# poriya219/modulations

Hardware: NVIDIA B200
Metric: turbo_info_throughput_N212_R1/3_8it (higher is better)
Workload: dtype f32/f64

## Files before the change

### modulations_b200/csrc/decode_tpf.cu

```cuda
#include "common.cuh"
#include "tpf_core.cuh"
#include "tpf_dev.cuh"

namespace b200dvb {

namespace {

using namespace tpf;

constexpr int kW = kTpfWin;

__device__ unsigned long long g_tpf_cycles[8];

struct TpfArgs {
    TpfGeom g;
    int B, iterations, n_tiles, n_llr, vec4;
    double sf_inner, sf_last;
    const int16_t *tab;
    const void *llr;
    long long llr_stride;
    int32_t *bits;
    uint32_t *packed;
    const uint8_t *ref_bits;
    unsigned long long *counters;
    unsigned char *ws;
    float llr_scale;
};

struct Ctx {
    int N, M, T;
    int f, isb, lane;
    unsigned tq;
    unsigned ycol;
    float4 *srec;
    unsigned char *stage;
    const int16_t *perm, *inv;
    float4 *L1A, *L2A;
    double2 *Le, *LeF, *Yb;
    float4 *CK;
    unsigned long long pol;
    unsigned one;
    __device__ __forceinline__ float4 *wstore() const { return reinterpret_cast<float4 *>(stage); }
    __device__ __forceinline__ float4 *slotZ() const { return reinterpret_cast<float4 *>(stage + 8192); }
    __device__ __forceinline__ float4 *slotX() const { return reinterpret_cast<float4 *>(stage + 10240); }
};

__device__ __forceinline__ void smem_get(const Ctx &c, int k, float (&g)[8])
{
    const float4 lo = c.srec[((k - c.T) * 2) * 16 + c.f], hi = c.srec[((k - c.T) * 2 + 1) * 16 + c.f];
    g[0] = lo.x; g[1] = lo.y; g[2] = lo.z; g[3] = lo.w; g[4] = hi.x; g[5] = hi.y; g[6] = hi.z; g[7] = hi.w;
}
__device__ __forceinline__ void smem_put(const Ctx &c, int k, const float (&g)[8])
{
    c.srec[((k - c.T) * 2) * 16 + c.f] = make_float4(g[0], g[1], g[2], g[3]);
    c.srec[((k - c.T) * 2 + 1) * 16 + c.f] = make_float4(g[4], g[5], g[6], g[7]);
}

struct Buf { float a[8], b[8]; };
template <int KIND> __device__ __forceinline__ void pf_issue(const Ctx &c, int j, Buf &B)
{
    if (KIND == 0) tm_ld8(c.tq + 8u * j, B.a);
    if (KIND == 1) smem_get(c, c.isb ? c.N - 1 - j : j, B.a);
    if (KIND == 2) {
        const unsigned col = 8u * (c.N - 1 - j);
        tm_ld8_half(c.tq + col, B.b);
        tm_ld8_half(c.tq + (16u << 16) + col, B.a);
    }
}
template <int KIND> __device__ __forceinline__ void pf_complete(const Ctx &c, Buf &B, float (&g)[8])
{
    if (KIND == 0) tm_wait_ld(B.a);
    if (KIND == 2) { tm_wait_ld(B.a); tm_wait_ld(B.b); }
#pragma unroll
    for (int i = 0; i < 8; ++i) g[i] = (KIND == 2 && c.isb) ? B.b[i] : B.a[i];
}

__device__ __forceinline__ constexpr int apos(int p) { return (p >> 1) | ((p & 1) << 3); }
__device__ __forceinline__ void pass_out(const Ctx &c, const float (&v)[16], float (&n)[16])
{
#pragma unroll
    for (int p = 0; p < 16; ++p) n[p] = c.isb ? v[rho4(p)] : v[apos(p)];
}
__device__ __forceinline__ void ck_store(const Ctx &c, int slot, const float (&v)[16])
{
    float n[16];
    pass_out(c, v, n);
#pragma unroll
    for (int q = 0; q < 4; ++q)
        st_ws(c.CK + (slot * 4 + q) * 32 + c.lane, make_float4(n[4 * q], n[4 * q + 1], n[4 * q + 2], n[4 * q + 3]));
}

template <int KIND, bool CK>
__device__ __forceinline__ void pass_two(const Ctx &c, int j, int j1, Buf &B0, Buf &B1, float (&g)[8], float (&v)[16])
{
    pf_issue<KIND>(c, j + 1, B1);
    if (CK) ck_store(c, (c.M - j) / kW - 1, v);
    pass_step(v, g, c.isb);
    pf_complete<KIND>(c, B1, g);
    pf_issue<KIND>(c, min(j + 2, j1 - 1), B0);
    pass_step(v, g, c.isb);
    pf_complete<KIND>(c, B0, g);
}
template <int KIND, bool CKA, bool CKB>
__device__ __forceinline__ void pass_loop(const Ctx &c, int j0, int j1, Buf &B0, Buf &B1, float (&g)[8], float (&v)[16])
{
    int j = j0;
    for (; j + 4 <= j1; j += 4) {
        pass_two<KIND, CKA>(c, j, j1, B0, B1, g, v);
        pass_two<KIND, CKB>(c, j + 2, j1, B0, B1, g, v);
    }
    if (j < j1) pass_two<KIND, CKA>(c, j, j1, B0, B1, g, v);
}
template <int KIND, bool CKPT>
__device__ __forceinline__ void run_pass(const Ctx &c, int j0, int j1, float (&v)[16])
{
    static_assert(kW == 4, "checkpoints alternate between the step pairs of a four-step body");
    if (j0 >= j1) return;
    Buf B0, B1;
    float g[8];
    pf_issue<KIND>(c, j0, B0);
    pf_complete<KIND>(c, B0, g);
    if (!CKPT) { pass_loop<KIND, false, false>(c, j0, j1, B0, B1, g, v); return; }
    if (j0 == 0 && (c.M % kW) != 0) ck_store(c, c.M / kW, v);
    if (((c.M - j0) % kW) == 0) pass_loop<KIND, CKPT, false>(c, j0, j1, B0, B1, g, v);
    else                        pass_loop<KIND, false, CKPT>(c, j0, j1, B0, B1, g, v);
}

__device__ __forceinline__ void issue_ckpt(const Ctx &c, int slot)
{
    float4 *dst = (c.isb ? c.slotZ() : c.slotX()) + c.lane;
#pragma unroll
    for (int q = 0; q < 4; ++q) cpa16(dst + q * 32, c.CK + (slot * 4 + q) * 32 + c.lane, c.one);
}
template <bool ALPHA = false>
__device__ __forceinline__ void slot_get(const float4 *slot, int lane, float (&v)[16])
{
    constexpr int P[4] = {ALPHA ? apos(0) : 0, ALPHA ? apos(1) : 1, ALPHA ? apos(2) : 2, ALPHA ? apos(3) : 3};
#pragma unroll
    for (int q = 0; q < 4; ++q) {
        const float4 t = slot[q * 32 + lane];
        const int b = ALPHA ? 2 * q : 4 * q;
        v[b + P[0]] = t.x; v[b + P[1]] = t.y; v[b + P[2]] = t.z; v[b + P[3]] = t.w;
    }
}
template <bool ALPHA = false>
__device__ __forceinline__ void slot_put(float4 *slot, int lane, const float (&v)[16])
{
    constexpr int P[4] = {ALPHA ? apos(0) : 0, ALPHA ? apos(1) : 1, ALPHA ? apos(2) : 2, ALPHA ? apos(3) : 3};
#pragma unroll
    for (int q = 0; q < 4; ++q) {
        const int b = ALPHA ? 2 * q : 4 * q;
        slot[q * 32 + lane] = make_float4(v[b + P[0]], v[b + P[1]], v[b + P[2]], v[b + P[3]]);
    }
}

__device__ __forceinline__ void st256_f64(void *p, double a, double b, double c, double d)
{
    asm volatile("st.global.cg.v4.f64 [%0], {%1,%2,%3,%4};" :: "l"(p), "d"(a), "d"(b), "d"(c), "d"(d) : "memory");
}
__device__ __forceinline__ void ld256_f64(const void *p, double2 &lo, double2 &hi)
{
    asm volatile("ld.global.cg.v4.f64 {%0,%1,%2,%3}, [%4];" : "=d"(lo.x), "=d"(lo.y), "=d"(hi.x), "=d"(hi.y) : "l"(p) : "memory");
}
__device__ __forceinline__ unsigned char *y_entry(const Ctx &c, int k_even)
{
    return reinterpret_cast<unsigned char *>(c.Yb) + ((size_t)(k_even >> 1) * 16 + c.f) * 32;
}
struct YQ { double2 y[kW]; };
__device__ __forceinline__ void yq_load(const Ctx &c, int w0, int len, YQ &q)
{
    static_assert(kW == 4, "two 32-byte entries per window");
    ld256_f64(y_entry(c, w0), q.y[0], q.y[1]);
    ld256_f64(y_entry(c, len > 2 ? w0 + 2 : w0), q.y[2], q.y[3]);
}
__device__ __forceinline__ void yq_park(const Ctx &c, const YQ &q, int w0, int len, int ck_slot)
{

#pragma unroll
    for (int u = 0; u < kW; ++u)
        asm volatile("tcgen05.st.sync.aligned.32x32b.x4.b32 [%0], {%1,%2,%3,%4};"
                     :: "r"(c.tq + c.ycol + 4u * u), "r"(__double2loint(q.y[u].x)), "r"(__double2hiint(q.y[u].x)),
                        "r"(__double2loint(q.y[u].y)), "r"(__double2hiint(q.y[u].y)) : "memory");
    tm_wait_st();
    const int dir = (c.lane >> 3) & 1, pr = (c.lane >> 2) & 1, l16 = c.lane & 15;
    const int w0d = __shfl_sync(0xffffffffu, w0, dir << 4);
    const void *line = c.lane < 16
        ? static_cast<const void *>(reinterpret_cast<const unsigned char *>(c.Yb) + ((size_t)((w0d >> 1) + pr) * 16) * 32 + (c.lane & 3) * 128)
        : static_cast<const void *>(c.CK + (ck_slot * 4 + (l16 >> 2)) * 32 + (l16 & 3) * 8);
    if (c.lane < 16 ? 2 * pr < len : ck_slot >= 0) l2_discard(line);
}

struct Pend { float uv[4], y[4]; int idx; };
__device__ __forceinline__ void pend_flush(const Ctx &c, Pend &p, double sf, double2 *LeOut)
{
    double ea, eb;
    make_extrinsic(p.uv, __hiloint2double(__float_as_int(p.y[1]), __float_as_int(p.y[0])),
                   __hiloint2double(__float_as_int(p.y[3]), __float_as_int(p.y[2])), sf, ea, eb);
    if (p.idx >= 0) st_ws(LeOut + p.idx * 16 + c.f, make_double2(ea, eb));
    p.idx = -1;
}
template <bool TM>
__device__ __forceinline__ void window(const Ctx &c, int wa, int w0, int len, double sf,
                                       double2 *LeOut, int nslot, int nw0, int nlen, Pend &pend)
{
    Buf B;
    auto issue = [&](int u) {
        if (TM) { tm_ld8(c.tq + 8u * (wa + u), B.a); tm_ld8(c.tq + 8u * (wa + len - 1 - u), B.b); }
        else    smem_get(c, w0 + u, B.a);
    };
    auto complete = [&](float (&g)[8]) {
        if (TM) { tm_wait_ld(B.a); tm_wait_ld(B.b); }
#pragma unroll
        for (int i = 0; i < 8; ++i) g[i] = (TM && c.isb) ? B.b[i] : B.a[i];
    };
    YQ nq;
    if (nlen) yq_load(c, nw0, nlen, nq);
    float g[8];
    float4 *ws = c.wstore() + c.lane;
    {
        float Z[16];
        issue(len - 1);
        slot_get(c.slotZ(), c.lane, Z);
        complete(g);
        slot_put(ws + (len - 1) * 128, 0, Z);
        issue(len - 2);
        pend_flush(c, pend, sf, LeOut);
        bwd_step(Z, g);
        complete(g);
        for (int u = len - 2; u >= 0; --u) {
            slot_put(ws + u * 128, 0, Z);
            issue(u > 0 ? u - 1 : 0);
            bwd_step(Z, g);
            complete(g);
        }
        if (!c.isb) slot_put(c.slotZ(), c.lane, Z);
    }
    float X[16];
    slot_get<true>(c.slotX(), c.lane, X);
    if (nslot >= 0) issue_ckpt(c, nslot);
    cpa_commit();
    float yr[4], yn[4], uvp[4], zs[16];
    tm_ld4(c.tq + c.ycol, yr);
    issue(len > 1 ? 1 : 0);
    slot_get(ws, 0, zs);
    ext_step(X, zs, g, uvp);
    tm_wait_ld4(yr);
    complete(g);
    for (int u = 1; u < len; ++u) {
        tm_ld4(c.tq + c.ycol + 4u * u, yn);
        issue(u + 1 < len ? u + 1 : u);
        slot_get(ws + u * 128, 0, zs);
        float uv[4];
        ext_step(X, zs, g, uv);
        double ea, eb;
        make_extrinsic(uvp, __hiloint2double(__float_as_int(yr[1]), __float_as_int(yr[0])),
                       __hiloint2double(__float_as_int(yr[3]), __float_as_int(yr[2])), sf, ea, eb);
        st_ws(LeOut + (w0 + u - 1) * 16 + c.f, make_double2(ea, eb));
        tm_wait_ld4(yn);
        complete(g);
#pragma unroll
        for (int i = 0; i < 4; ++i) { uvp[i] = uv[i]; yr[i] = yn[i]; }
    }
#pragma unroll
    for (int i = 0; i < 4; ++i) { pend.uv[i] = uvp[i]; pend.y[i] = yr[i]; }
    pend.idx = w0 + len - 1;
    if (c.isb) slot_put<true>(c.slotX(), c.lane, X);
    if (nlen) yq_park(c, nq, nw0, nlen, nslot - 1);
}


__device__ __forceinline__ int lpos(const Ctx &c, int k, int fr) { return k < c.M ? k * 32 + fr : (c.N - 1 - k) * 32 + 16 + fr; }

struct Idx { int a, b; };
__device__ __forceinline__ void idx_get(const Ctx &c, int jn, const int16_t *tbl, Idx &x)
{
    jn = min(jn, c.M - 2);
    const int k0 = c.isb ? c.N - 1 - jn : jn, k1 = c.isb ? k0 - 1 : k0 + 1;
    x.a = tbl[k0]; x.b = tbl[k1];
}
__device__ __forceinline__ void prep_load_pair(const Ctx &c, unsigned char *slot, int jn, const float4 *Lsrc,
                                               const Idx &x, bool first)
{
    jn = min(jn, c.M - 2);
    const unsigned d = s_addr(slot) * c.one;
    const float4 *src = Lsrc + jn * 32 + c.lane;
    cpa16_stream_off<0, 0>(d, src, c.pol);
    cpa16_stream_off<1024, 512>(d, src, c.pol);
    if (!first) {
        cpa16_off<512, 0>(d, c.Le + x.a * 16 + c.f);
        cpa16_off<1536, 0>(d, c.Le + x.b * 16 + c.f);
    }
}
struct Raw { float4 xA, xB; double2 laA, laB; };
template <bool FIRST>
__device__ __forceinline__ void raw_get(const unsigned char *slot, Raw &r)
{
    r.xA = *reinterpret_cast<const float4 *>(slot);
    r.xB = *reinterpret_cast<const float4 *>(slot + 1024);
    r.laA = r.laB = make_double2(0.0, 0.0);
    if (!FIRST) {
        r.laA = *reinterpret_cast<const double2 *>(slot + 512);
        r.laB = *reinterpret_cast<const double2 *>(slot + 1536);
    }
}
struct PrepRec { float gA[8], gB[8]; };
__device__ __forceinline__ void prep_pair(const Ctx &c, const Raw &r, int jn, PrepRec &out)
{
    jn = min(jn, c.M - 2);
    const double2 YA = make_double2(d_add((double)r.xA.x, r.laA.x), d_add((double)r.xA.y, r.laA.y));
    const double2 YB = make_double2(d_add((double)r.xB.x, r.laB.x), d_add((double)r.xB.y, r.laB.y));
    make_record(YA.x, YA.y, r.xA.z, r.xA.w, out.gA);
    make_record(YB.x, YB.y, r.xB.z, r.xB.w, out.gB);
#ifndef TPF_ABL_NOY
    const int ke = c.isb ? c.N - 2 - jn : jn;
    st256_f64(y_entry(c, ke), c.isb ? YB.x : YA.x, c.isb ? YB.y : YA.y, c.isb ? YA.x : YB.x, c.isb ? YA.y : YB.y);
#endif
}
struct PrepState { PrepRec r; Raw raw; Idx ix; int ps; };
template <bool FIRST, bool TMST>
__device__ __forceinline__ void pass1a_pair(const Ctx &c, int jj, const float4 *Lsrc, const int16_t *tbl,
                                            int &ps, const PrepRec &in, PrepRec &out, const Raw &rin, Raw &rout,
                                            const Idx &xin, Idx &xout, float (&v)[16])
{
    const int N = c.N;
    unsigned char *slot = c.stage + c.lane * 16 + ps * 2048;
    cpa_wait<kRingPairs - 1>();
#ifndef TPF_ABL_NORAW
    raw_get<FIRST>(slot, rout);
#else
    rout = rin;
#endif
#ifndef TPF_ABL_NOCPA
    prep_load_pair(c, slot, jj + 4 + 2 * kRingPairs, Lsrc, xin, FIRST);
    cpa_commit();
    if (!FIRST) idx_get(c, jj + 6 + 2 * kRingPairs, tbl, xout);
#endif
    ps = ps == kRingPairs - 1 ? 0 : ps + 1;
#ifndef TPF_ABL_NOFP64
    prep_pair(c, rin, jj + 2, out);
#else
    out = in;
#endif
    const int k0 = c.isb ? N - 1 - jj : jj, k1 = c.isb ? N - 2 - jj : jj + 1;
#ifndef TPF_ABL_NOREC
    if (TMST) tm_st8(c.tq + 8u * jj, in.gA);
    else      smem_put(c, k0, in.gA);
#endif
    pass_step(v, in.gA, c.isb);
#ifndef TPF_ABL_NOREC
    if (TMST) tm_st8(c.tq + 8u * (jj + 1), in.gB);
    else      smem_put(c, k1, in.gB);
#endif
    pass_step(v, in.gB, c.isb);
}
template <bool FIRST, bool TMST>
__device__ __forceinline__ void pass1a_range(const Ctx &c, int j0, int j1, const float4 *Lsrc,
                                             const int16_t *tbl, PrepState &P, float (&v)[16])
{
    PrepRec Q;
    Raw RQ;
    Idx XQ = P.ix;
    int jj = j0;
    for (; jj + 4 <= j1; jj += 4) {
        pass1a_pair<FIRST, TMST>(c, jj, Lsrc, tbl, P.ps, P.r, Q, P.raw, RQ, P.ix, XQ, v);
        pass1a_pair<FIRST, TMST>(c, jj + 2, Lsrc, tbl, P.ps, Q, P.r, RQ, P.raw, XQ, P.ix, v);
    }
    if (jj < j1) {
        pass1a_pair<FIRST, TMST>(c, jj, Lsrc, tbl, P.ps, P.r, Q, P.raw, RQ, P.ix, XQ, v);
        P.r = Q;
        P.raw = RQ;
        P.ix = XQ;
    }
}

template <bool FIRST>
__device__ __forceinline__ void pass1a(const Ctx &c, bool second, float (&v)[16])
{
    const float4 *Lsrc = second ? c.L2A : c.L1A;
    const int16_t *tbl = second ? c.perm : c.inv;
    unsigned char *ring = c.stage + c.lane * 16;
    PrepState P;
    P.ix.a = P.ix.b = 0;
#pragma unroll 1
    for (int p = 0; p < kRingPairs; ++p) {
        if (!FIRST) idx_get(c, 2 * p, tbl, P.ix);
        prep_load_pair(c, ring + p * 2048, 2 * p, Lsrc, P.ix, FIRST);
        cpa_commit();
    }
    if (!FIRST) idx_get(c, 2 * kRingPairs, tbl, P.ix);
    cpa_wait<kRingPairs - 1>();
    raw_get<FIRST>(ring, P.raw);
    prep_pair(c, P.raw, 0, P.r);
    prep_load_pair(c, ring, 2 * kRingPairs, Lsrc, P.ix, FIRST);
    cpa_commit();
    if (!FIRST) idx_get(c, 2 * kRingPairs + 2, tbl, P.ix);
    cpa_wait<kRingPairs - 1>();
    raw_get<FIRST>(ring + 2048, P.raw);
    prep_load_pair(c, ring + 2048, 2 * kRingPairs + 2, Lsrc, P.ix, FIRST);
    cpa_commit();
    if (!FIRST) idx_get(c, 2 * kRingPairs + 4, tbl, P.ix);
    P.ps = 2 % kRingPairs;
    pass1a_range<FIRST, true>(c, 0, c.T, Lsrc, tbl, P, v);
    pass1a_range<FIRST, false>(c, c.T, c.M, Lsrc, tbl, P, v);
    cpa_wait<0>();
}

template <bool TIMED>
__device__ __forceinline__ void siso(const Ctx &c, bool second, bool first, bool last, double sf, long long (&ph)[8])
{
    long long tA = TIMED ? clock64() : 0;
    const int N = c.N, M = c.M, T = c.T, lane = c.lane;
    double2 *LeOut = last ? c.LeF : c.Le;
    float v[16];
#pragma unroll
    for (int s = 0; s < 16; ++s) v[s] = 0.f;
    if (first) pass1a<true>(c, second, v);
    else       pass1a<false>(c, second, v);
    tm_wait_st();
    __syncwarp();
    if (!first && !last)
        for (int i = lane; i < N * 2; i += 32) l2_discard(c.Le + i * 8);
    if (TIMED) { const long long t = clock64(); ph[1] += t - tA; tA = t; }
    run_pass<1, false>(c, M, N - T, v);
    run_pass<2, false>(c, N - T, N, v);
    if (TIMED) { const long long t = clock64(); ph[2] += t - tA; tA = t; }
    const int nfull = M / kW, rag = M % kW, nwin = nfull + (rag ? 1 : 0);
    auto win_w0 = [&](int i) { return i < nfull ? (c.isb ? M + i * kW : M - (i + 1) * kW) : (c.isb ? N - rag : 0); };
    auto win_len = [&](int i) { return i < nfull ? kW : rag; };
    {
        YQ q0;
        yq_load(c, win_w0(0), win_len(0), q0);
        run_pass<0, true>(c, 0, T, v);
        run_pass<1, true>(c, T, M, v);
        yq_park(c, q0, win_w0(0), win_len(0), -1);
    }
    if (TIMED) { const long long t = clock64(); ph[3] += t - tA; tA = t; }
    {
        float n[16];
        pass_out(c, v, n);
        slot_put(c.isb ? c.slotZ() : c.slotX(), lane ^ 16, n);
    }
    const int n_inner = (M - T) / kW;
    issue_ckpt(c, 0);
    cpa_commit();
    Pend pend;
#pragma unroll
    for (int i = 0; i < 4; ++i) pend.uv[i] = pend.y[i] = 0.f;
    pend.idx = -1;
    for (int i = 0; i < nwin; ++i) {
        cpa_wait<0>();
        __syncwarp();
        const int wa = i < nfull ? M - (i + 1) * kW : 0;
        const int nlen = i + 1 < nwin ? win_len(i + 1) : 0;
        const int nw0 = i + 1 < nwin ? win_w0(i + 1) : 0;
        if (i < n_inner) window<false>(c, wa, win_w0(i), win_len(i), sf, LeOut, nlen ? i + 1 : -1, nw0, nlen, pend);
        else             window<true>(c, wa, win_w0(i), win_len(i), sf, LeOut, nlen ? i + 1 : -1, nw0, nlen, pend);
        if (TIMED && i == n_inner - 1) { const long long t = clock64(); ph[4] += t - tA; tA = t; }
    }
    pend_flush(c, pend, sf, LeOut);
    cpa_wait<0>();
    __syncwarp();
    if (TIMED) { const long long t = clock64(); ph[5] += t - tA; tA = t; }
}

template <bool TIMED, class LlrT>
__global__ void __launch_bounds__(kTpfWarps * 32, 1)
tpf_kernel(const TpfArgs A)
{
    extern __shared__ __align__(16) unsigned char smem_raw[];
    const TpfGeom g = A.g;
    const int N = g.N;
    const int tid = threadIdx.x, lane = tid & 31, warp = tid >> 5;
    int16_t *tab = reinterpret_cast<int16_t *>(smem_raw);
    const int tab_bytes = ((2 * N * 2 + 15) / 16) * 16;
    unsigned *tmem_slot = reinterpret_cast<unsigned *>(smem_raw + tab_bytes);
    float4 *srec_all = reinterpret_cast<float4 *>(smem_raw + tab_bytes + 64);
    unsigned char *stage_all = reinterpret_cast<unsigned char *>(srec_all + (size_t)kTpfWarps * g.mid * 2 * 16);
    if (warp == 0) {
        asm volatile("tcgen05.alloc.cta_group::1.sync.aligned.shared::cta.b32 [%0], %1;"
                     ::"r"((unsigned)__cvta_generic_to_shared(tmem_slot)), "r"(g.tmem_cols) : "memory");
        asm volatile("tcgen05.relinquish_alloc_permit.cta_group::1.sync.aligned;" ::: "memory");
    }
    for (int i = tid; i < 2 * N; i += blockDim.x) tab[i] = A.tab[i];
    const unsigned mbar = (unsigned)__cvta_generic_to_shared(smem_raw + tab_bytes + 32 + 8 * warp);
    unsigned mphase = 0;
    if (lane == 0) { mbar_init(mbar, 1); mbar_fence_init(); }
    asm volatile("tcgen05.fence::before_thread_sync;" ::: "memory");
    __syncthreads();
    asm volatile("tcgen05.fence::after_thread_sync;" ::: "memory");
    const unsigned tmem_base = *tmem_slot;

    Ctx c;
    c.N = N; c.M = g.M; c.T = g.T;
    c.f = lane & 15; c.isb = lane >> 4; c.lane = lane;
    c.tq = tmem_base + (((unsigned)warp * 32u) << 16);
    c.ycol = 8u * g.T;
    c.srec = srec_all + (size_t)warp * g.mid * 2 * 16;
    {
        volatile unsigned *slots = reinterpret_cast<volatile unsigned *>(smem_raw + tab_bytes);
        if (lane == 0) { slots[4 + warp] = (unsigned)warp * kStageBytes; slots[1] = 1u; }
        __syncwarp();
        c.stage = stage_all + slots[4 + warp];
        c.one = slots[1];
        __syncwarp();
    }
    c.perm = tab; c.inv = tab + N;
    const int wg = blockIdx.x * kTpfWarps + warp;
    unsigned char *ws = A.ws + (size_t)wg * g.ws_per_warp;
    c.L1A = reinterpret_cast<float4 *>(ws + g.off_l1);
    c.L2A = reinterpret_cast<float4 *>(ws + g.off_l2);
    c.Le = reinterpret_cast<double2 *>(ws + g.off_le);
    c.LeF = reinterpret_cast<double2 *>(ws + g.off_lef);
    c.Yb = reinterpret_cast<double2 *>(ws + g.off_y);
    c.CK = reinterpret_cast<float4 *>(ws + g.off_ck);
    asm volatile("createpolicy.fractional.L2::evict_first.b64 %0, 1.0;" : "=l"(c.pol));
    const int16_t *g_off = A.tab + 2 * N;

    unsigned long long bit_err = 0, frm_err = 0, frames_done = 0;
    long long ph[8] = {0, 0, 0, 0, 0, 0, 0, 0};
    const long long t_begin = TIMED ? clock64() : 0;
    for (int tile = wg; tile < A.n_tiles; tile += gridDim.x * kTpfWarps) {
        const long long frame0 = (long long)tile * kTpfFrames;
        const long long t0 = TIMED ? clock64() : 0;
        const float sc = A.llr_scale;
        if (A.vec4) {
            const int nq = llr_row_q<LlrT>(A.n_llr);
            const int pitch4 = ((nq + 6) & ~7) + 1;
            const int rec_bytes = g.mid * 2 * 16 * (int)sizeof(float4);
            const bool in_rec = rec_bytes > kStageBytes;
            float4 *rowbuf = in_rec ? c.srec : reinterpret_cast<float4 *>(c.stage);
            const int fit = (in_rec ? rec_bytes : kStageBytes - N * 16) / (pitch4 * 16);
            const int lg = fit >= 8 ? 3 : fit >= 4 ? 2 : 1, G = 1 << lg, KQ = 32 >> lg;
            const int fr = lane & (G - 1), kq = lane >> lg;
            int4 *otab = reinterpret_cast<int4 *>(in_rec ? c.stage : c.stage + G * pitch4 * 16);
            for (int k = lane; k < N; k += 32) {
                const unsigned oa = (unsigned short)__ldg(g_off + k), op = (unsigned short)__ldg(g_off + c.perm[k]);
                const unsigned o0 = (unsigned short)__ldg(g_off + N + k), o1 = (unsigned short)__ldg(g_off + 2 * N + k);
                const unsigned o2 = (unsigned short)__ldg(g_off + 3 * N + k), o3 = (unsigned short)__ldg(g_off + 4 * N + k);
                otab[k] = make_int4((int)(oa | (op << 16)), (int)(o0 | (o1 << 16)), (int)(o2 | (o3 << 16)), 0);
            }
            auto pull = [&](int g0) {
                if (lane == 0) {
                    int live_rows = 0;
                    for (int r = 0; r < G; ++r) live_rows += frame0 + g0 + r < A.B;
                    fence_proxy_async();
                    mbar_expect_tx(mbar, (unsigned)(live_rows * nq * 16));
                    for (int r = 0; r < live_rows; ++r)
                        bulk_g2s_stream(rowbuf + r * pitch4, static_cast<const LlrT *>(A.llr) + (frame0 + g0 + r) * A.llr_stride, (unsigned)(nq * 16), mbar, c.pol);
                }
            };
            pull(0);
            if (A.ref_bits) {
                const int lines = (2 * N * kTpfFrames + 127) / 128;
                const long long nb = min((long long)kTpfFrames, A.B - frame0) * 2 * N;
                for (int i = lane; i < lines; i += 32)
                    if ((long long)i * 128 < nb) asm volatile("prefetch.global.L2 [%0];" ::"l"(A.ref_bits + frame0 * 2 * N + i * 128));
            }
            const LlrT *row = reinterpret_cast<const LlrT *>(rowbuf + fr * pitch4);
            for (int g0 = 0; g0 < kTpfFrames; g0 += G) {
                mbar_wait(mbar, mphase);
                mphase ^= 1u;
                const bool livef = frame0 + g0 + fr < A.B;
#pragma unroll 4
                for (int k0 = 0; k0 < N; k0 += KQ) {
                    const int k = k0 + kq;
                    const int4 e = otab[min(k, N - 1)];
                    const int oa = (short)(e.x & 0xffff), op = e.x >> 16, o0 = (short)(e.y & 0xffff), o1 = e.y >> 16;
                    const int o2 = (short)(e.z & 0xffff), o3 = e.z >> 16;
                    float4 x1 = make_float4(0.f, 0.f, 0.f, 0.f), x2 = x1;
                    if (livef) {
                        x1.x = llr_f32(row[oa], sc); x1.y = llr_f32(row[oa + 1], sc); x2.x = llr_f32(row[op], sc); x2.y = llr_f32(row[op + 1], sc);
                        if (o0 >= 0) x1.z = llr_f32(row[o0], sc);
                        if (o1 >= 0) x1.w = llr_f32(row[o1], sc);
                        if (o2 >= 0) x2.z = llr_f32(row[o2], sc);
                        if (o3 >= 0) x2.w = llr_f32(row[o3], sc);
                    }
                    if (k < N) {
                        st_ws(c.L1A + lpos(c, k, g0 + fr), x1);
                        st_ws(c.L2A + lpos(c, k, g0 + fr), x2);
                    }
                }
                __syncwarp();
                if (g0 + G < kTpfFrames) pull(g0 + G);
            }
        } else
        for (int k = lane; k < N; k += 32) {
            const int oa = __ldg(g_off + k), op = __ldg(g_off + c.perm[k]);
            const int o0 = __ldg(g_off + N + k), o1 = __ldg(g_off + 2 * N + k);
            const int o2 = __ldg(g_off + 3 * N + k), o3 = __ldg(g_off + 4 * N + k);
#pragma unroll
            for (int f0 = 0; f0 < kTpfFrames; f0 += 8) {
                float4 x1[8], x2[8];
#pragma unroll
                for (int fr = 0; fr < 8; ++fr) {
                    const long long frame = frame0 + f0 + fr;
                    const LlrT *Lf = static_cast<const LlrT *>(A.llr) + frame * A.llr_stride;
                    x1[fr] = make_float4(0.f, 0.f, 0.f, 0.f); x2[fr] = x1[fr];
                    if (frame < A.B) {
                        x1[fr].x = llr_ldg(Lf + oa, sc); x1[fr].y = llr_ldg(Lf + oa + 1, sc);
                        x2[fr].x = llr_ldg(Lf + op, sc); x2[fr].y = llr_ldg(Lf + op + 1, sc);
                        if (o0 >= 0) x1[fr].z = llr_ldg(Lf + o0, sc);
                        if (o1 >= 0) x1[fr].w = llr_ldg(Lf + o1, sc);
                        if (o2 >= 0) x2[fr].z = llr_ldg(Lf + o2, sc);
                        if (o3 >= 0) x2[fr].w = llr_ldg(Lf + o3, sc);
                    }
                }
#pragma unroll
                for (int fr = 0; fr < 8; ++fr) {
                    st_ws(c.L1A + lpos(c, k, f0 + fr), x1[fr]);
                    st_ws(c.L2A + lpos(c, k, f0 + fr), x2[fr]);
                }
            }
        }
        __syncwarp();
        if (TIMED) ph[0] += clock64() - t0;
        for (int h = 0; h < 2 * A.iterations; ++h) {
            const double sf = (h >> 1) < A.iterations - 1 ? A.sf_inner : A.sf_last;
            siso<TIMED>(c, (h & 1) != 0, h == 0, h == 2 * A.iterations - 1, sf, ph);
        }
        const long long t6 = TIMED ? clock64() : 0;
        const long long frame = frame0 + c.f;
        const bool live = frame < A.B;
        const int wpf = (2 * N + 31) / 32;
        const bool cnt = live && A.ref_bits != nullptr;
        const uint8_t *refp = cnt ? A.ref_bits + (size_t)frame * 2 * N : reinterpret_cast<const uint8_t *>(A.tab);
        constexpr int kHB = 3 * 8 * 32 * 16;
        const int rec_bytes_h = g.mid * 2 * 16 * (int)sizeof(float4);
        unsigned char *hbuf = rec_bytes_h >= kHB ? reinterpret_cast<unsigned char *>(c.srec) : c.stage;
        const int nst = rec_bytes_h >= 3 * kHB ? 3 : rec_bytes_h >= 2 * kHB ? 2 : 1;
        const int nwords = (N + 15) / 16;
        const int nbu = 2 * ((nwords + 1) / 2);
        auto hissue = [&](int b, int st) {
            if (b < nbu) {
                const int kb = (c.isb + 2 * (b >> 1)) * 16 + 8 * (b & 1);
                const unsigned d = s_addr(hbuf + st * kHB + lane * 16) * c.one;
#pragma unroll
                for (int t = 0; t < 8; ++t) {
                    const int k = min(kb + t, N - 1);
                    const unsigned dt = d + t * 512;
                    cpa16_off<0, 0>(dt, c.L1A + lpos(c, k, c.f));
                    cpa16_off<4096, 0>(dt, c.LeF + c.inv[k] * 16 + c.f);
                    cpa16_off<8192, 0>(dt, c.Le + k * 16 + c.f);
                }
            }
            cpa_commit();
        };
        int any_err = 0;
        unsigned word = 0;
        for (int b = 0; b < nst; ++b) hissue(b, b);
        for (int b = 0, st = 0; b < nbu; ++b) {
            if (nst == 3) cpa_wait<2>(); else if (nst == 2) cpa_wait<1>(); else cpa_wait<0>();
            const int kb = (c.isb + 2 * (b >> 1)) * 16 + 8 * (b & 1);
            const unsigned char *src = hbuf + st * kHB + lane * 16;
            unsigned short rb[8];
#pragma unroll
            for (int t = 0; t < 8; ++t) rb[t] = *reinterpret_cast<const unsigned short *>(refp + 2 * min(kb + t, N - 1));
#pragma unroll
            for (int t = 0; t < 8; ++t) {
                const int k = kb + t;
                const float4 ab = *reinterpret_cast<const float4 *>(src + t * 512);
                const double2 la = *reinterpret_cast<const double2 *>(src + 4096 + t * 512);
                const double2 e1 = *reinterpret_cast<const double2 *>(src + 8192 + t * 512);
                const double LA = d_add(d_add((double)ab.x, la.x), e1.x);
                const double LB = d_add(d_add((double)ab.y, la.y), e1.y);
                const int bA = LA < 0.0, bB = LB < 0.0;
                if (k < N) {
                    word |= (unsigned)(bA | (bB << 1)) << (2 * (8 * (b & 1) + t));
                    if (live && A.bits)
                        *reinterpret_cast<int2 *>(A.bits + (size_t)frame * 2 * N + 2 * k) = make_int2(bA, bB);
                    if (cnt) {
                        const int errs = (bA != (rb[t] & 0xff)) + (bB != (rb[t] >> 8));
                        bit_err += errs;
                        any_err |= errs;
                    }
                }
            }
            hissue(b + nst, st);
            st = st + 1 == nst ? 0 : st + 1;
            if (b & 1) {
                const int w = c.isb + b - 1;
                if (live && A.packed && w < nwords) A.packed[(size_t)frame * wpf + w] = word;
                word = 0;
            }
        }
        cpa_wait<0>();
        any_err |= __shfl_xor_sync(0xffffffffu, any_err, 16);
        if (live && !c.isb) { frames_done += 1; frm_err += any_err ? 1 : 0; }
        __syncwarp();
        if (TIMED) ph[6] += clock64() - t6;
    }
    if (TIMED && lane == 0) {
        ph[7] = clock64() - t_begin;
        for (int i = 0; i < 8; ++i) atomicAdd(&g_tpf_cycles[i], (unsigned long long)ph[i]);
    }
    if (A.counters) {
        for (int o = 16; o > 0; o >>= 1) {
            bit_err += __shfl_xor_sync(0xffffffffu, bit_err, o);
            frm_err += __shfl_xor_sync(0xffffffffu, frm_err, o);
            frames_done += __shfl_xor_sync(0xffffffffu, frames_done, o);
        }
        if (lane == 0) {
            if (bit_err) atomicAdd(A.counters + 0, bit_err);
            if (frm_err) atomicAdd(A.counters + 1, frm_err);
            if (frames_done) {
                atomicAdd(A.counters + 2, frames_done);
                atomicAdd(A.counters + 3, frames_done * 2ull * N);
            }
        }
    }
    asm volatile("tcgen05.fence::before_thread_sync;" ::: "memory");
    __syncthreads();
    if (warp == 0)
        asm volatile("tcgen05.dealloc.cta_group::1.sync.aligned.b32 %0, %1;" ::"r"(tmem_base), "r"(g.tmem_cols) : "memory");
}

}

void tpf_family_geometry(TpfGeom &g, int N, int y_cols, size_t hdr_bytes, size_t ext_bytes, bool with_init, size_t smem_optin)
{
    g = TpfGeom{};
    if (N < 16 || (N % 4) != 0) return;
    const int M = N / 2;
    int T = M < 64 ? M : 64;
    while (T > 0 && (((M - T) % kW) != 0 || 8 * T + y_cols > 512)) --T;
    if (T < kW) return;
    g.N = N; g.M = M; g.T = T; g.mid = N - 2 * T;
    g.nfull = M / kW; g.rag = M % kW; g.nslots = g.nfull + (g.rag ? 1 : 0);
    g.tmem_cols = 32;
    while (g.tmem_cols < 8 * T + y_cols) g.tmem_cols *= 2;
    if (g.tmem_cols > 512) return;
    const size_t tab_bytes = ((size_t)2 * N * 2 + 15) / 16 * 16;
    g.smem_bytes = tab_bytes + hdr_bytes + (size_t)kTpfWarps * g.mid * 2 * 16 * sizeof(float4) + (size_t)kTpfWarps * kStageBytes;
    if (g.smem_bytes > smem_optin) return;
    size_t off = 0;
    auto take = [&](size_t bytes) { const size_t o = off; off += (bytes + 255) / 256 * 256; return o; };
    g.off_l1 = take((size_t)N * 16 * sizeof(float4));
    g.off_l2 = take((size_t)N * 16 * sizeof(float4));
    g.off_le = take((size_t)N * 16 * ext_bytes);
    g.off_lef = take((size_t)N * 16 * ext_bytes);
    g.off_y = take((size_t)N * 16 * ext_bytes);
    g.off_ck = take((size_t)g.nslots * 4 * 32 * sizeof(float4));
    if (with_init) g.off_init = take((size_t)2 * 4 * 32 * sizeof(float4));
    g.ws_per_warp = off;
    g.enabled = 1;
}

int tpf_family_grid(const Codec &c, int B, int tile)
{
    const int tiles = (B + tile - 1) / tile;
    const int ctas = (tiles + kTpfWarps - 1) / kTpfWarps;
    return ctas < c.num_sms ? ctas : c.num_sms;
}

size_t tpf_family_workspace_bytes(const Codec &c, const TpfGeom &g, int B, int tile)
{
    return (size_t)tpf_family_grid(c, B, tile) * kTpfWarps * g.ws_per_warp + 256;
}

int tpf_family_row_staging(const Codec &c, const TpfGeom &g, const DecodeIo &io)
{
    const int nq = llr_row_q(io.fmt, c.n_llr);
    if (c.N > 256 || (io.llr_stride * llr_bytes(io.fmt)) % 16 != 0 || (reinterpret_cast<uintptr_t>(io.llr) & 15) != 0 ||
        nq * 4 > kRowFloats || c.opt_no_row_staging)
        return 0;
    const int pitch4 = ((nq + 6) & ~7) + 1;
    const int rec_bytes = g.mid * 2 * 16 * (int)sizeof(float4);
    const int avail = rec_bytes > kStageBytes ? rec_bytes : kStageBytes - c.N * 16;
    return avail / (pitch4 * 16) >= 2;
}

int tpf_configure(Codec &c, size_t smem_optin)
{
    tpf_family_geometry(c.tpf, c.N, 4 * kW, 64, sizeof(double2), false, smem_optin);
    if (!c.tpf.enabled) return B200DVB_OK;
    return for_each_llr_type([&](auto t) {
        using L = decltype(t);
        B2_CUDA(cudaFuncSetAttribute(tpf_kernel<false, L>, cudaFuncAttributeMaxDynamicSharedMemorySize, (int)smem_optin));
        B2_CUDA(cudaFuncSetAttribute(tpf_kernel<true, L>, cudaFuncAttributeMaxDynamicSharedMemorySize, (int)smem_optin));
        return B200DVB_OK;
    });
}

int tpf_read_phase_cycles(double *out_h, int reset) { return read_phase_cycles(g_tpf_cycles, out_h, reset); }

size_t tpf_workspace_bytes(const Codec &c, int B) { return tpf_family_workspace_bytes(c, c.tpf, B, kTpfFrames); }

int tpf_launch_decode(const Codec &c, const DecodeIo &io)
{
    if (io.ws_bytes < tpf_workspace_bytes(c, io.B)) return B200DVB_ENOMEM;
    TpfArgs A{};
    fill_decode_args(A, c, io);
    A.g = c.tpf;
    A.n_tiles = (io.B + kTpfFrames - 1) / kTpfFrames;
    A.n_llr = c.n_llr;
    A.vec4 = tpf_family_row_staging(c, c.tpf, io);
    A.ws = reinterpret_cast<unsigned char *>((reinterpret_cast<uintptr_t>(io.ws) + 255) & ~(uintptr_t)255);
    const int grid = tpf_family_grid(c, io.B, kTpfFrames);
    const bool timed = c.opt_phase_timers != 0;
    with_llr_type(io.fmt, [&](auto t) {
        using L = decltype(t);
        if (timed) tpf_kernel<true, L><<<grid, kTpfWarps * 32, c.tpf.smem_bytes, io.stream>>>(A);
        else       tpf_kernel<false, L><<<grid, kTpfWarps * 32, c.tpf.smem_bytes, io.stream>>>(A);
    });
    B2_CUDA(cudaGetLastError());
    return B200DVB_OK;
}

}
```

Measured before the change: 4.059.

## Deepen prefetch pipeline in turbo decoder passes and unroll smem window loads

Restructures the forward/backward pass loop from two rotating buffers into a four-buffer ring, one step per stage. The shared-memory path now prefetches two steps ahead and the TMEM paths one step ahead, with waits split from register moves. The shared-memory index is precomputed as a per-lane base pointer and signed stride, replacing per-step branch and arithmetic. The non-TMEM window backward sweep is fully unrolled for a fixed window length, loading all four records up front. The aim is to hide load latency in the serial recursion, at the cost of more registers and occupancy risk.

```diff
diff --git a/modulations_b200/csrc/decode_tpf.cu b/modulations_b200/csrc/decode_tpf.cu
--- a/modulations_b200/csrc/decode_tpf.cu
+++ b/modulations_b200/csrc/decode_tpf.cu
@@ -33,6 +33,8 @@
     unsigned tq;
     unsigned ycol;
     float4 *srec;
+    const float4 *srec_j;
+    int srec_dj;
     unsigned char *stage;
     const int16_t *perm, *inv;
     float4 *L1A, *L2A;
@@ -60,17 +62,23 @@
 template <int KIND> __device__ __forceinline__ void pf_issue(const Ctx &c, int j, Buf &B)
 {
     if (KIND == 0) tm_ld8(c.tq + 8u * j, B.a);
-    if (KIND == 1) smem_get(c, c.isb ? c.N - 1 - j : j, B.a);
+    if (KIND == 1) {
+        const float4 lo = c.srec_j[j * c.srec_dj], hi = c.srec_j[j * c.srec_dj + 16];
+        B.a[0] = lo.x; B.a[1] = lo.y; B.a[2] = lo.z; B.a[3] = lo.w; B.a[4] = hi.x; B.a[5] = hi.y; B.a[6] = hi.z; B.a[7] = hi.w;
+    }
     if (KIND == 2) {
         const unsigned col = 8u * (c.N - 1 - j);
         tm_ld8_half(c.tq + col, B.b);
         tm_ld8_half(c.tq + (16u << 16) + col, B.a);
     }
 }
-template <int KIND> __device__ __forceinline__ void pf_complete(const Ctx &c, Buf &B, float (&g)[8])
-{
-    if (KIND == 0) tm_wait_ld(B.a);
-    if (KIND == 2) { tm_wait_ld(B.a); tm_wait_ld(B.b); }
+template <int KIND> __device__ __forceinline__ void pf_complete(Buf &B)
+{
+    if (KIND != 1) tm_wait_ld(B.a);
+    if (KIND == 2) tm_wait_ld(B.b);
+}
+template <int KIND> __device__ __forceinline__ void pf_rec(const Ctx &c, const Buf &B, float (&g)[8])
+{
 #pragma unroll
     for (int i = 0; i < 8; ++i) g[i] = (KIND == 2 && c.isb) ? B.b[i] : B.a[i];
 }
@@ -90,40 +98,52 @@
         st_ws(c.CK + (slot * 4 + q) * 32 + c.lane, make_float4(n[4 * q], n[4 * q + 1], n[4 * q + 2], n[4 * q + 3]));
 }
 
-template <int KIND, bool CK>
-__device__ __forceinline__ void pass_two(const Ctx &c, int j, int j1, Buf &B0, Buf &B1, float (&g)[8], float (&v)[16])
-{
-    pf_issue<KIND>(c, j + 1, B1);
+template <int KIND> constexpr int kPfDist = KIND == 1 ? 2 : 1;
+template <int KIND, bool CK, int S>
+__device__ __forceinline__ void pass_one(const Ctx &c, int j, int j1, Buf (&B)[4], float (&v)[16])
+{
+    constexpr int D = kPfDist<KIND>;
+    pf_complete<KIND>(B[S]);
+    pf_issue<KIND>(c, (D == 2 || (S & 1)) ? min(j + D, j1 - 1) : j + D, B[(S + D) & 3]);
     if (CK) ck_store(c, (c.M - j) / kW - 1, v);
+    float g[8];
+    pf_rec<KIND>(c, B[S], g);
     pass_step(v, g, c.isb);
-    pf_complete<KIND>(c, B1, g);
-    pf_issue<KIND>(c, min(j + 2, j1 - 1), B0);
-    pass_step(v, g, c.isb);
-    pf_complete<KIND>(c, B0, g);
 }
 template <int KIND, bool CKA, bool CKB>
-__device__ __forceinline__ void pass_loop(const Ctx &c, int j0, int j1, Buf &B0, Buf &B1, float (&g)[8], float (&v)[16])
+__device__ __forceinline__ void pass_loop(const Ctx &c, int j0, int j1, Buf (&B)[4], float (&v)[16])
 {
     int j = j0;
     for (; j + 4 <= j1; j += 4) {
-        pass_two<KIND, CKA>(c, j, j1, B0, B1, g, v);
-        pass_two<KIND, CKB>(c, j + 2, j1, B0, B1, g, v);
-    }
-    if (j < j1) pass_two<KIND, CKA>(c, j, j1, B0, B1, g, v);
+        pass_one<KIND, CKA, 0>(c, j, j1, B, v);
+        pass_one<KIND, false, 1>(c, j + 1, j1, B, v);
+        pass_one<KIND, CKB, 2>(c, j + 2, j1, B, v);
+        pass_one<KIND, false, 3>(c, j + 3, j1, B, v);
+    }
+    if (j < j1) {
+        pass_one<KIND, CKA, 0>(c, j, j1, B, v);
+        pass_one<KIND, false, 1>(c, j + 1, j1, B, v);
+    }
 }
 template <int KIND, bool CKPT>
 __device__ __forceinline__ void run_pass(const Ctx &c, int j0, int j1, float (&v)[16])
 {
     static_assert(kW == 4, "checkpoints alternate between the step pairs of a four-step body");
     if (j0 >= j1) return;
-    Buf B0, B1;
-    float g[8];
-    pf_issue<KIND>(c, j0, B0);
-    pf_complete<KIND>(c, B0, g);
-    if (!CKPT) { pass_loop<KIND, false, false>(c, j0, j1, B0, B1, g, v); return; }
-    if (j0 == 0 && (c.M % kW) != 0) ck_store(c, c.M / kW, v);
-    if (((c.M - j0) % kW) == 0) pass_loop<KIND, CKPT, false>(c, j0, j1, B0, B1, g, v);
-    else                        pass_loop<KIND, false, CKPT>(c, j0, j1, B0, B1, g, v);
+    Buf B[4];
+    pf_issue<KIND>(c, j0, B[0]);
+    if (kPfDist<KIND> == 2) pf_issue<KIND>(c, j0 + 1, B[1]);
+    if (!CKPT) pass_loop<KIND, false, false>(c, j0, j1, B, v);
+    else {
+        if (j0 == 0 && (c.M % kW) != 0) ck_store(c, c.M / kW, v);
+        if (((c.M - j0) % kW) == 0) pass_loop<KIND, CKPT, false>(c, j0, j1, B, v);
+        else                        pass_loop<KIND, false, CKPT>(c, j0, j1, B, v);
+    }
+    if (KIND != 1) {
+        tm_wait_ld(B[0].a);
+        tm_wait_ld(B[2].a);
+        if (KIND == 2) { tm_wait_ld(B[0].b); tm_wait_ld(B[2].b); }
+    }
 }
 
 __device__ __forceinline__ void issue_ckpt(const Ctx &c, int slot)
@@ -217,7 +237,22 @@
     if (nlen) yq_load(c, nw0, nlen, nq);
     float g[8];
     float4 *ws = c.wstore() + c.lane;
-    {
+    if (!TM) {
+        float G[kW][8], Z[16];
+#pragma unroll
+        for (int u = 0; u < kW; ++u) smem_get(c, w0 + u, G[u]);
+        slot_get(c.slotZ(), c.lane, Z);
+        slot_put(ws + (kW - 1) * 128, 0, Z);
+        pend_flush(c, pend, sf, LeOut);
+#pragma unroll
+        for (int u = kW - 1; u >= 0; --u) {
+            if (u < kW - 1) slot_put(ws + u * 128, 0, Z);
+            bwd_step(Z, G[u]);
+        }
+#pragma unroll
+        for (int i = 0; i < 8; ++i) g[i] = G[0][i];
+        if (!c.isb) slot_put(c.slotZ(), c.lane, Z);
+    } else {
         float Z[16];
         issue(len - 1);
         slot_get(c.slotZ(), c.lane, Z);
@@ -496,6 +531,8 @@
     c.tq = tmem_base + (((unsigned)warp * 32u) << 16);
     c.ycol = 8u * g.T;
     c.srec = srec_all + (size_t)warp * g.mid * 2 * 16;
+    c.srec_j = c.srec + ((c.isb ? N - 1 : 0) - g.T) * 32 + c.f;
+    c.srec_dj = c.isb ? -32 : 32;
     {
         volatile unsigned *slots = reinterpret_cast<volatile unsigned *>(smem_raw + tab_bytes);
         if (lane == 0) { slots[4 + warp] = (unsigned)warp * kStageBytes; slots[1] = 1u; }
```

Result: faster. 4.210, median of 6 (+3.7%).
